# jolars/sgdnet

Measured on AMD Instinct MI355X. Metric: saga_epochs_per_sec, higher is better.
Workload: dtype f64

## Files before the change

### sgdnet_amd/csrc/saga_batched.hip

```cpp
#include <hip/hip_ext.h>
#include <stdlib.h>

#include <mutex>
#include <set>
#include <type_traits>
#include <utility>

#include "device_math.hpp"
#include "r_rng_word.hpp"
#include "r_rng_bodies.hpp"

#ifndef SGDNET_BIN_BLOCK
#define SGDNET_BIN_BLOCK 1024
#endif
#ifndef SGDNET_BIN_W
#define SGDNET_BIN_W 8
#endif
#ifndef SGDNET_RANGE_BLOCK
#define SGDNET_RANGE_BLOCK 512
#endif

namespace sgdnet {

namespace {
// ... 1615 lines not shown
  const int E = F * K;
  const int v = (int)blockIdx.x / nfb, fb = (int)blockIdx.x - v * nfb;
  const int64_t KP = (int64_t)K * d.p;
  const double n_d = d.v_size[v];
  const int e = threadIdx.x % kSlabElems, g = threadIdx.x / kSlabElems;
  const int64_t elem = (int64_t)fb * E + e;
  const int64_t j_own = (int64_t)fb * F + threadIdx.x;
  const bool updates = (int)threadIdx.x < F && j_own < d.p;
  double w_old[KMAX], g_old[KMAX], c_own = 0.0;
#pragma unroll
  for (int k = 0; k < KMAX; ++k) {
    w_old[k] = g_old[k] = 0.0;
    if (updates && k < K) {
      w_old[k] = d.vw[(int64_t)v * KP + j_own * K + k];
      g_old[k] = d.vG[(int64_t)v * KP + j_own * K + k];
    }
  }
  if (updates && d.standardize) c_own = d.c[j_own];
  double acc = 0.0;
  if (e < E && elem < KP) {
    const double* sp = d.slab + (int64_t)v * d.v_bps * KP + elem;
    int bidx = g;
    for (; bidx + 3 * kSlabGroups < d.v_bps; bidx += 4 * kSlabGroups) {
      const double a0 = sp[(int64_t)bidx * KP], a1 = sp[(int64_t)(bidx + kSlabGroups) * KP];
      const double a2 = sp[(int64_t)(bidx + 2 * kSlabGroups) * KP];
      const double a3 = sp[(int64_t)(bidx + 3 * kSlabGroups) * KP];
      acc += (a0 + a1) + (a2 + a3);
    }
    for (; bidx < d.v_bps; bidx += kSlabGroups) acc += sp[(int64_t)bidx * KP];
  }
  part[g][e] = acc;
  const bool need_d0 = fb == 0 || d.standardize;
  if (need_d0) {
    for (int k = 0; k < K; ++k) {
      double a = 0.0;
      for (int i = threadIdx.x; i < d.v_bps; i += kBlock) a += d.vd0[(int64_t)(v * d.v_bps + i) * K + k];
      a = wave_sum(a);
      if ((threadIdx.x & 63) == 0) red[threadIdx.x >> 6] = a;
      __syncthreads();
      if (threadIdx.x == 0) {
        double t = 0.0;
        for (int wv = 0; wv < kBlock / 64; ++wv) t += red[wv];
        sh_d0[k] = t;
      }
      __syncthreads();
    }
  } else {
    __syncthreads();
  }
  if (updates) {
    double dj[KMAX], val[KMAX];
#pragma unroll
    for (int k = 0; k < KMAX; ++k) {
      dj[k] = 0.0;
      if (k < K) {
        const int ee = (int)threadIdx.x * K + k;
        double t = 0.0;
        for (int gg = 0; gg < kSlabGroups; ++gg) t += part[gg][ee];
        dj[k] = t - (d.standardize ? c_own * sh_d0[k] : 0.0);
      }
    }
    const double gls = q.gamma * q.ls_m;
    double nrm = 0.0;
#pragma unroll
    for (int k = 0; k < KMAX; ++k) {
      val[k] = k < K ? q.r_m * w_old[k] - gls * g_old[k] - q.gamma * dj[k] : 0.0;
      nrm += val[k] * val[k];
    }
    const double tau = q.beta * q.gamma * q.ls_m;
    const double factor = q.penalty == SGDNET_GROUPLASSO ? tau / sqrt(nrm) : 0.0;
#pragma unroll
    for (int k = 0; k < KMAX; ++k) {
      if (k < K) {
        double out = val[k];
        if (q.penalty == SGDNET_ELASTICNET) out = soft_threshold(out, tau);
        else if (q.penalty == SGDNET_GROUPLASSO) out = factor < 1.0 ? out * (1.0 - factor) : 0.0;
        d.vw[(int64_t)v * KP + j_own * K + k] = out;
        if (dj[k] != 0.0 || q.penalty == SGDNET_GROUPLASSO)
          d.vG[(int64_t)v * KP + j_own * K + k] = g_old[k] + dj[k] / n_d;
      }
    }
  }
  if (fb == 0 && (int)threadIdx.x < K && d.fit_intercept) {
    const int k = threadIdx.x;
    const double dk = sh_d0[k] / n_d;
    const double gbk = d.vgb[v * K + k] + dk;
    d.vgb[v * K + k] = gbk;
    d.vb[v * K + k] -= q.gamma * (gbk * (d.xd ? 1.0 : 0.01) * q.m_d + dk);
  }
}

__global__ __launch_bounds__(kBlock) void saga_vs_cw_kernel(SagaDev d) {
  __shared__ double red[kBlock / 64];
  const int K = d.K;
  const int v = (int)blockIdx.x / K, k = (int)blockIdx.x - v * K;
  const double* wv = d.vw + (int64_t)v * K * d.p + k;
  double a = 0.0;
  for (int64_t j = threadIdx.x; j < d.p; j += kBlock) a += d.c[j] * wv[j * K];
  a = wave_sum(a);
  if ((threadIdx.x & 63) == 0) red[threadIdx.x >> 6] = a;
  __syncthreads();
  if (threadIdx.x == 0) {
    double t = 0.0;
    for (int wvi = 0; wvi < kBlock / 64; ++wvi) t += red[wvi];
    d.vcw[blockIdx.x] = t;
  }
}

__device__ __forceinline__ double* vs_slot(const SagaDev& d, int v, int64_t i, int64_t KP, int K) {
  if (i < KP) return d.vG + (int64_t)v * KP + i;
  if (i < 2 * KP) return d.vw + (int64_t)v * KP + (i - KP);
  if (i < 2 * KP + K) return d.vgb + (int64_t)v * K + (i - 2 * KP);
  return d.vb + (int64_t)v * K + (i - 2 * KP - K);
}
__device__ __forceinline__ double* vs_own_slot(const SagaDev& d, int64_t i, int64_t KP, int K) {
  if (i < KP) return d.G + i;
  if (i < 2 * KP) return d.w + (i - KP);
  if (i < 2 * KP + K) return d.gb + (i - 2 * KP);
  return d.b + (i - 2 * KP - K);
}

__global__ __launch_bounds__(kBlock) void saga_vs_broadcast_kernel(SagaDev d) {
  const int K = d.K;
  const int64_t KP = (int64_t)K * d.p, len = 2 * KP + 2 * K;
  for (int64_t i = (int64_t)blockIdx.x * kBlock + threadIdx.x; i < len; i += (int64_t)gridDim.x * kBlock) {
    const double val = *vs_own_slot(d, i, KP, K);
    d.vref[i] = val;
    for (int v = 0; v < d.V; ++v) *vs_slot(d, v, i, KP, K) = val;
  }
}

__global__ __launch_bounds__(kBlock) void saga_vs_merge_kernel(SagaDev d, int final_merge, LamParams* epoch_end,
                                                               int batches) {
  if (epoch_end && blockIdx.x == 0 && threadIdx.x == 0) end_epoch(epoch_end, batches);
  const int K = d.K;
  const int64_t KP = (int64_t)K * d.p, len = 2 * KP + 2 * K;
  double tot_size = 0.0;
  for (int v = 0; v < d.V; ++v) tot_size += d.v_size[v];
  for (int64_t i = (int64_t)blockIdx.x * kBlock + threadIdx.x; i < len; i += (int64_t)gridDim.x * kBlock) {
    const double ref = d.vref[i];
    double val = ref;
    for (int v = 0; v < d.V; ++v) val += (d.v_size[v] / tot_size) * (*vs_slot(d, v, i, KP, K) - ref);
    d.vref[i] = val;
    for (int v = 0; v < d.V; ++v) *vs_slot(d, v, i, KP, K) = val;
    if (final_merge) *vs_own_slot(d, i, KP, K) = val;
  }
}

__global__ void saga_epoch_end_kernel(LamParams* lamp, int batches) {
  if (threadIdx.x == 0 && blockIdx.x == 0) end_epoch(lamp, batches);
}

constexpr int kSyncLine = 32;
constexpr int kSyncGo = 0, kSyncExit = 1, kSyncStart = 2, kSyncCnt1 = 3, kSyncCnt2 = kSyncCnt1 + 8,
              kSyncXcd = kSyncCnt2 + 8;
constexpr int kFusedMaxBps = 128;
constexpr int kSyncLines = kSyncXcd + 8;
constexpr int kSyncSticky = kSyncLines;
constexpr int kSyncSeq = kSyncLines + 1;
constexpr int kFusedChunks = 3;
constexpr long long kFusedStartTicks = 2000000;
constexpr long long kFusedWaitTicks = 200000000;

typedef unsigned int u32x4_t __attribute__((ext_vector_type(4)));
typedef double f64x2_t __attribute__((ext_vector_type(2)));

__device__ __forceinline__ __amdgpu_buffer_rsrc_t fused_rsrc(const void* base, int64_t bytes) {
  return __builtin_amdgcn_make_buffer_rsrc(const_cast<void*>(base), 0, (int)bytes, 0x00020000);
}
__device__ __forceinline__ void st2_sc1(f64x2_t x, __amdgpu_buffer_rsrc_t rs, uint32_t byte_off) {
  __builtin_amdgcn_raw_buffer_store_b128(__builtin_bit_cast(u32x4_t, x), rs, (int)byte_off, 0, 16);
}
__device__ __forceinline__ f64x2_t ld2_sc1(__amdgpu_buffer_rsrc_t rs, uint32_t byte_off) {
  return __builtin_bit_cast(f64x2_t, __builtin_amdgcn_raw_buffer_load_b128(rs, (int)byte_off, 0, 16));
}
__device__ __forceinline__ void st2_shard(f64x2_t x, __amdgpu_buffer_rsrc_t rs, uint32_t byte_off, bool local) {
  if (local)
    __builtin_amdgcn_raw_buffer_store_b128(__builtin_bit_cast(u32x4_t, x), rs, (int)byte_off, 0, 0);
  else
    __builtin_amdgcn_raw_buffer_store_b128(__builtin_bit_cast(u32x4_t, x), rs, (int)byte_off, 0, 16);
}
__device__ __forceinline__ void st_shard(double* q, double x, bool local) {
  if (local)
    *q = x;
  else
    __hip_atomic_store(q, x, __ATOMIC_RELAXED, __HIP_MEMORY_SCOPE_AGENT);
}
__device__ __forceinline__ void st_sc1(double* q, double x) {
  __hip_atomic_store(q, x, __ATOMIC_RELAXED, __HIP_MEMORY_SCOPE_AGENT);
}
__device__ __forceinline__ double ld_sc1(const double* q) {
  return __hip_atomic_load(q, __ATOMIC_RELAXED, __HIP_MEMORY_SCOPE_AGENT);
}
__device__ __forceinline__ void st_sys(double* q, double x) {
  __hip_atomic_store(q, x, __ATOMIC_RELAXED, __HIP_MEMORY_SCOPE_SYSTEM);
}
__device__ __forceinline__ double ld_sys(const double* q) {
  return __hip_atomic_load(q, __ATOMIC_RELAXED, __HIP_MEMORY_SCOPE_SYSTEM);
}
__device__ __forceinline__ unsigned sync_load(unsigned* sync, int word) {
  return __hip_atomic_load(sync + word * kSyncLine, __ATOMIC_RELAXED, __HIP_MEMORY_SCOPE_AGENT);
}

__device__ __forceinline__ void fused_arrive(unsigned* sync, int word) {
  asm volatile("s_waitcnt vmcnt(0)" ::: "memory");
  __syncthreads();
  if (threadIdx.x == 0)
    __hip_atomic_fetch_add(sync + word * kSyncLine, 1u, __ATOMIC_RELAXED, __HIP_MEMORY_SCOPE_AGENT);
}

__device__ __forceinline__ bool fused_poll(unsigned* ctr, int word, unsigned target, LamParams* lamp, bool system = false,
                                           unsigned* sync = nullptr) {
  if (!sync) sync = ctr;
  const long long t0 = wall_clock64();
  for (unsigned spins = 1;; ++spins) {
    const unsigned now = system ? __hip_atomic_load(ctr + word * kSyncLine, __ATOMIC_RELAXED, __HIP_MEMORY_SCOPE_SYSTEM)
                                : sync_load(ctr, word);
    if (now >= target) return true;
    __builtin_amdgcn_s_sleep(4);
    if ((spins & 63u) == 0) {
      if (sync_load(sync, kSyncGo) != 1u) return false;
      if (wall_clock64() - t0 > kFusedWaitTicks) {
        __hip_atomic_store(sync + kSyncGo * kSyncLine, 3u, __ATOMIC_RELAXED, __HIP_MEMORY_SCOPE_AGENT);
        __hip_atomic_store(&lamp->fused_abort, 2, __ATOMIC_RELAXED, __HIP_MEMORY_SCOPE_AGENT);
        __hip_atomic_store(sync + kSyncSticky * kSyncLine, 2u, __ATOMIC_RELAXED, __HIP_MEMORY_SCOPE_AGENT);
        return false;
      }
    }
  }
}

__device__ __forceinline__ bool fused_start(unsigned* sync, LamParams* lamp, unsigned grid) {
  unsigned* go = sync + kSyncGo * kSyncLine;
  const long long t0 = wall_clock64();
  if (blockIdx.x == 0) {
    unsigned expect = 0u;
    for (;;) {
      if (sync_load(sync, kSyncStart) >= grid) {
        __hip_atomic_compare_exchange_strong(go, &expect, 1u, __ATOMIC_RELAXED, __ATOMIC_RELAXED, __HIP_MEMORY_SCOPE_AGENT);
        break;
      }
      if (sync_load(sync, kSyncGo) != 0u) break;
      if (wall_clock64() - t0 > kFusedStartTicks) {
        __hip_atomic_compare_exchange_strong(go, &expect, 2u, __ATOMIC_RELAXED, __ATOMIC_RELAXED, __HIP_MEMORY_SCOPE_AGENT);
        break;
      }
      __builtin_amdgcn_s_sleep(4);
    }
  } else {
    for (;;) {
      if (sync_load(sync, kSyncGo) != 0u) break;
      if (wall_clock64() - t0 > 2 * kFusedStartTicks) {
        unsigned expect = 0u;
        __hip_atomic_compare_exchange_strong(go, &expect, 2u, __ATOMIC_RELAXED, __ATOMIC_RELAXED, __HIP_MEMORY_SCOPE_AGENT);
        break;
      }
      __builtin_amdgcn_s_sleep(4);
    }
  }
  const unsigned decision = sync_load(sync, kSyncGo);
  if (decision != 1u && decision != 3u) {
    __hip_atomic_store(&lamp->fused_abort, 1, __ATOMIC_RELAXED, __HIP_MEMORY_SCOPE_AGENT);
    __hip_atomic_fetch_max(sync + kSyncSticky * kSyncLine, 1u, __ATOMIC_RELAXED, __HIP_MEMORY_SCOPE_AGENT);
  }
  return decision == 1u;
}

__device__ __forceinline__ double fused_block_sum(double a, double* red) {
  a = wave_sum(a);
  if ((threadIdx.x & 63) == 0) red[threadIdx.x >> 6] = a;
  __syncthreads();
  double t = 0.0;
#pragma unroll
  for (int wv = 0; wv < kLdsBlock / 64; ++wv) t += red[wv];
  __syncthreads();
  return t;
}

__device__ __forceinline__ void fused_leave(const SagaDev& d, LamParams* lamp, int nb, bool epoch_done) {
  asm volatile("s_waitcnt vmcnt(0)" ::: "memory");
  __syncthreads();
  if (threadIdx.x == 0) {
    unsigned* sync = d.vsync;
    if (epoch_done && blockIdx.x == 0) {
      end_epoch(lamp, nb);
      if (d.n_peers > 1) __hip_atomic_fetch_add(sync + kSyncSeq * kSyncLine, 1u, __ATOMIC_RELAXED, __HIP_MEMORY_SCOPE_AGENT);
    }
    const unsigned prev = __hip_atomic_fetch_add(sync + kSyncExit * kSyncLine, 1u, __ATOMIC_RELAXED, __HIP_MEMORY_SCOPE_AGENT);
    if (prev + 1u == gridDim.x) {
      for (int wd = 0; wd < kSyncLines; ++wd)
        __hip_atomic_store(sync + wd * kSyncLine, 0u, __ATOMIC_RELAXED, __HIP_MEMORY_SCOPE_AGENT);
      if (!(d.n_peers > 1))
        for (int wd = 0; wd < kFusedMaxBps; ++wd)
          __hip_atomic_store(d.vcol + wd * kSyncLine, 0u, __ATOMIC_RELAXED, __HIP_MEMORY_SCOPE_AGENT);
      if (d.rngdev && lamp->rng_generate) d.rngdev->gen += 1u;
    }
  }
}

template <bool kPeers>
__global__ __launch_bounds__(kLdsBlock) void saga_vs_epoch_kernel(SagaDev d, LamParams* lamp, int nb, int every) {
  extern __shared__ __attribute__((aligned(16))) double Dl[];
  __shared__ int ticket_counter;
  __shared__ int sh_ok;
  __shared__ double sh_red[kLdsBlock / 64];
  __shared__ double sh_val[4];
  const int tid = threadIdx.x;
  const int64_t p = d.p;
  const int64_t P2 = p >> 1;
  const int S = d.v_bps, V = d.V;
  if ((int)blockIdx.x >= V * S) {
    if (d.rngdev && lamp->rng_generate) {
      const RngDev* R = d.rngdev;
      const unsigned gen = R->gen;
      uint32_t* lds = reinterpret_cast<uint32_t*>(Dl);
      const int rb = (int)blockIdx.x - V * S, nrb = (int)gridDim.x - V * S;
      mt_state_body(rb, nrb, reinterpret_cast<uint32_t(*)[2][kMtN + 1]>(lds), R->state[gen & 1u], R->ends,
                    R->stream + (int64_t)(gen & 1u) * R->n, R->n, R->seg, R->gens);
      __syncthreads();
      mt_jump_body(rb, nrb, lds, R->state[gen & 1u], R->state[(gen + 1u) & 1u], R->poly, R->gens);
    }
    fused_leave(d, lamp, nb, false);
    return;
  }
  const int v = (int)blockIdx.x % V, wi = (int)blockIdx.x / V;
  const int F = 2 * (int)((p + 2 * S - 1) / (2 * S));
  const int j0 = wi * F;
  const int jn = p - j0 < F ? (p - j0 > 0 ? (int)(p - j0) : 0) : F;
  double* Wl = Dl + p;
  f64x2_t* D2 = reinterpret_cast<f64x2_t*>(Dl);
  f64x2_t* W2 = reinterpret_cast<f64x2_t*>(Wl);
  const int penalty = lamp->penalty;
  __shared__ double sh_par[10];
  if (tid == 0) {
    sh_par[0] = lamp->gamma;
    sh_par[1] = lamp->beta;
    sh_par[2] = lamp->r_full;
    sh_par[3] = lamp->ls_full;
    sh_par[4] = lamp->r_tail;
    sh_par[5] = lamp->ls_tail;
    double tot = 0.0, lo = 0.0;
    for (int u = 0; u < d.V; ++u) {
      tot += d.v_size[u];
      if (u < (int)blockIdx.x % d.V) lo += d.v_size[u];
    }
    sh_par[6] = d.v_size[(int)blockIdx.x % d.V];
    sh_par[7] = lo;
    sh_par[8] = tot;
  }
  const int64_t m_full = lamp->m_full;
  const int64_t sbase = lamp->stream_base;
  const bool raw_words = lamp->stream_raw != 0;
  const int64_t dps = d.v_dps;
  const bool std_x = d.standardize != 0;
  const int64_t L = 2 * p + 2;
  double* vwv = d.vw + (int64_t)v * p;
  double* vGv = d.vG + (int64_t)v * p;
  double* refv = d.vx + (int64_t)v * L;
  double* cwp = d.vx + (int64_t)V * L;
  unsigned* sync = d.vsync;
  const __amdgpu_buffer_rsrc_t rs_slab = fused_rsrc(d.slab, (int64_t)V * S * p * 8);
  const __amdgpu_buffer_rsrc_t rs_w = fused_rsrc(vwv, p * 8);
  uint32_t* const stream_v = const_cast<uint32_t*>(d.stream) + sbase + (int64_t)v * dps;
  constexpr int kC = 8;
  auto conv_range = [&](int m, int& lo, int& hi) {
    const int share = ((m + S - 1) / S + kTicket - 1) / kTicket * kTicket;
    lo = wi * share;
    hi = lo + share < m ? lo + share : m;
  };
  auto conv_load = [&](int64_t t0, int m, uint32_t (&x)[kC]) {
    int lo, hi;
    conv_range(m, lo, hi);
    const uint32_t* q = stream_v + t0;
#pragma unroll
    for (int c = 0; c < kC; ++c) {
      const int i = lo + (int)threadIdx.x + c * kLdsBlock;
      x[c] = i < hi ? q[i] : 0u;
    }
  };
  auto conv_store = [&](int64_t t0, int m, const uint32_t (&x)[kC]) {
    int lo, hi;
    conv_range(m, lo, hi);
    uint32_t* q = stream_v + t0;
    const double n_d = sh_par[6], lo_v = sh_par[7];
#pragma unroll
    for (int c = 0; c < kC; ++c) {
      const int i = lo + (int)threadIdx.x + c * kLdsBlock;
      if (i < hi) q[i] = (uint32_t)lo_v + word_to_draw(x[c], n_d);
    }
    for (int i = lo + (int)threadIdx.x + kC * kLdsBlock; i < hi; i += kLdsBlock)
      q[i] = (uint32_t)lo_v + word_to_draw(q[i], n_d);
  };

#ifdef SGDNET_PHASE_TIMING
  unsigned long long ph_t = 0;
  if (d.dbg && tid == 0) d.dbg[(size_t)blockIdx.x * 16 + 14] = ph_t = phase_stamp();
#define FPH(slot)                                                 \
  do {                                                            \
    if (d.dbg && tid == 0) {                                      \
      const unsigned long long now = phase_stamp();               \
      d.dbg[(size_t)blockIdx.x * 16 + (slot)] += now - ph_t;      \
      d.dbg[(size_t)blockIdx.x * 16 + 15] = ph_t = now;           \
    }                                                             \
  } while (0)
#else
#define FPH(slot) ((void)0)
#endif
  if (tid == 0) {
    const unsigned xcc = __builtin_amdgcn_s_getreg((3 << 11) | 20) & 15u;
    __hip_atomic_fetch_or(sync + (kSyncXcd + v) * kSyncLine, 1u << xcc, __ATOMIC_RELAXED, __HIP_MEMORY_SCOPE_AGENT);
    asm volatile("s_waitcnt vmcnt(0)" ::: "memory");
    __hip_atomic_fetch_add(sync + kSyncStart * kSyncLine, 1u, __ATOMIC_RELAXED, __HIP_MEMORY_SCOPE_AGENT);
    sh_ok = fused_start(sync, lamp, (unsigned)(V * S)) ? 1 : 0;
    if (sh_ok) {
      const unsigned mask = sync_load(sync, kSyncXcd + v);
      sh_ok = (mask & (mask - 1u)) == 0u ? 3 : 1;
    }
  }
  for (int64_t i = tid; i < P2; i += kLdsBlock) D2[i] = f64x2_t{0.0, 0.0};
  __syncthreads();
  bool done = false;
  bool alive = sh_ok != 0;
  unsigned col_base = 0u;
  if (kPeers) {
    int merges = 0;
    for (int r = 0; r < nb; ++r) merges += (r + 1 == nb || (r + 1) % every == 0) ? 1 : 0;
    col_base = sync_load(sync, kSyncSeq) * (unsigned)merges;
  }
  const bool local = (sh_ok & 2) != 0 && d.vs_xcd_local != 0;
  int mi = 0;
  uint32_t s_first = 0u, s_second = 0u;
  if (alive) {
    const int m0 = (int)(dps < m_full ? dps : m_full);
    if (raw_words) {
      uint32_t x0[kC];
      conv_load(0, m0, x0);
      conv_store(0, m0, x0);
      asm volatile("s_waitcnt vmcnt(0)" ::: "memory");
      __syncthreads();
    }
    K1Compact nx;
    nx.begin(d, stream_v, m0, wi, S, &ticket_counter);
    s_first = nx.s_cur;
    s_second = nx.s_nxt;
  }
  for (int r = 0; alive && r < nb; ++r) {
    const int64_t t0 = (int64_t)r * m_full;
    const int m = (int)(dps - t0 < m_full ? dps - t0 : m_full);
    const bool tail = m != m_full;
    const bool last = r + 1 == nb;
    const bool merge_due = last || (r + 1) % every == 0;

    if (tid == 0) ticket_counter = K1Compact::static_tickets();
    K1Compact cg;
    cg.init(d, stream_v + t0, m, wi, S, &ticket_counter);
    cg.s_cur = s_first;
    cg.s_nxt = s_second;
    cg.tag_first();
    int ts = threadIdx.x;
    asm volatile("" : "+v"(ts));
    double cw = 0.0, bv = 0.0;
    if ((ts >> 6) == 0) {
      if (std_x && r > 0)
        for (int k = ts & 63; k < S; k += 64) cw += ld_sc1(cwp + v * kFusedMaxBps + k);
      bv = r == 0 ? d.b[0] : ld_sc1(d.vb + v);
    }
    {
      constexpr int kStage = 8;
      for (int64_t i0 = ts; i0 < P2; i0 += (int64_t)kLdsBlock * kStage) {
        f64x2_t t[kStage];
#pragma unroll
        for (int q = 0; q < kStage; ++q) {
          const int64_t i = i0 + (int64_t)q * kLdsBlock;
          t[q] = f64x2_t{0.0, 0.0};
          if (i < P2) t[q] = r == 0 ? reinterpret_cast<const f64x2_t*>(d.w)[i] : ld2_sc1(rs_w, (uint32_t)(i * 16));
        }
#pragma unroll
        for (int q = 0; q < kStage; ++q) {
          const int64_t i = i0 + (int64_t)q * kLdsBlock;
          if (i < P2) W2[i] = t[q];
        }
      }
    }
    if ((ts >> 6) == 0) {
      cw = wave_sum(cw);
      if ((ts & 63) == 0) sh_val[0] = bv - cw;
    }
    __syncthreads();
    if (r == 0 && std_x) {
      double a = 0.0;
      for (int64_t j = ts; j < p; j += kLdsBlock) a += d.c[j] * Wl[j];
      a = fused_block_sum(a, sh_red);
      if (ts == 0) sh_val[0] -= a;
      __syncthreads();
    }
    const double b0 = sh_val[0];
    FPH(0);

    const double gct = cg.run(d, b0, Wl, Dl);
    __syncthreads();
    FPH(1);
    int tq = threadIdx.x;
    asm volatile("" : "+v"(tq));
    const int lane = tq & 63, wave = tq >> 6;
    const int64_t t0n = t0 + m_full;
    const int mn = (int)(dps - t0n < m_full ? dps - t0n : m_full);
    uint32_t xraw[kC];
    const bool conv_next = !last && raw_words;

    {
      const uint32_t base = (uint32_t)(((int64_t)blockIdx.x * p) * 8);
      for (int64_t i = tq; i < P2; i += kLdsBlock) {
        st2_shard(D2[i], rs_slab, base + (uint32_t)(i * 16), local);
        D2[i] = f64x2_t{0.0, 0.0};
      }
      const double t = wave_sum(gct);
      if (lane == 0) sh_red[wave] = t;
      __syncthreads();
      if (tq == 0) {
        double tot = 0.0;
        for (int wv = 0; wv < kLdsBlock / 64; ++wv) tot += sh_red[wv];
        st_shard(d.vd0 + blockIdx.x, tot, local);
      }
    }
    fused_arrive(sync, kSyncCnt1 + v);
    FPH(2);
    if (conv_next) conv_load(t0n, mn, xraw);
    const bool upd = tq < jn;
    const bool icpt = wi == 0 && tq == jn;
    const bool act = upd || icpt;
    const int64_t j = j0 + tq;
    const int64_t oa = upd ? j : 2 * p, ob = upd ? p + j : 2 * p + 1;
    double* const rep_a = upd ? vGv + j : d.vgb + v;
    double* const rep_b = upd ? vwv + j : d.vb + v;
    const double* const own_a = upd ? d.G + j : d.gb;
    const double* const own_b = upd ? d.w + j : d.b;
    double a_old = 0.0, b_old = 0.0, c_own = 0.0, ra = 0.0, rb = 0.0;
    if (act) {
      a_old = r == 0 ? *own_a : ld_sc1(rep_a);
      b_old = r == 0 ? *own_b : ld_sc1(rep_b);
      if (std_x && upd) c_own = d.c[j];
      if (merge_due) {
        ra = mi == 0 ? *own_a : ld_sc1(refv + oa);
        rb = mi == 0 ? *own_b : ld_sc1(refv + ob);
      }
    }
    if (tq == 0) sh_ok = fused_poll(sync, kSyncCnt1 + v, (unsigned)S * (unsigned)(r + 1), lamp) ? 1 : 0;
    __syncthreads();
    if (!sh_ok) break;
    FPH(3);
    if (conv_next) conv_store(t0n, mn, xraw);

    {
      double gsum = 0.0;
      if (wave == kLdsBlock / 64 - 1)
        for (int k = lane; k < S; k += 64) gsum += ld_sc1(d.vd0 + k * V + v);
      f64x2_t acc[kFusedChunks];
#pragma unroll
      for (int c = 0; c < kFusedChunks; ++c) acc[c] = f64x2_t{0.0, 0.0};
      for (int k = wave; k < S; k += 2 * (kLdsBlock / 64)) {
        const bool two = k + kLdsBlock / 64 < S;
        const uint32_t o0 = (uint32_t)((((int64_t)(k * V + v)) * p + j0) * 8);
        const uint32_t o1 = (uint32_t)((((int64_t)((k + kLdsBlock / 64) * V + v)) * p + j0) * 8);
        f64x2_t a0[kFusedChunks], a1[kFusedChunks];
#pragma unroll
        for (int c = 0; c < kFusedChunks; ++c) {
          const int pi = c * 64 + lane;
          a0[c] = a1[c] = f64x2_t{0.0, 0.0};
          if (2 * pi < jn) {
            a0[c] = ld2_sc1(rs_slab, o0 + (uint32_t)(pi * 16));
            if (two) a1[c] = ld2_sc1(rs_slab, o1 + (uint32_t)(pi * 16));
          }
        }
#pragma unroll
        for (int c = 0; c < kFusedChunks; ++c) {
          acc[c] += a0[c];
          acc[c] += a1[c];
        }
      }
#pragma unroll
      for (int c = 0; c < kFusedChunks; ++c) {
        const int pi = c * 64 + lane;
        if (2 * pi < F) reinterpret_cast<f64x2_t*>(Wl + (int64_t)wave * F)[pi] = acc[c];
      }
      if (wave == kLdsBlock / 64 - 1) {
        gsum = wave_sum(gsum);
        if (lane == 0) sh_val[1] = gsum;
      }
    }
    __syncthreads();
    double a_new = a_old, b_new = b_old;
    {
      const double d0 = sh_val[1];
      const double n_d = sh_par[6], gamma = sh_par[0];
      if (upd) {
        double dj = 0.0;
#pragma unroll
        for (int wv = 0; wv < kLdsBlock / 64; ++wv) dj += Wl[(int64_t)wv * F + tq];
        if (std_x) dj -= c_own * d0;
        const double beta = sh_par[1];
        const double r_m = tail ? sh_par[4] : sh_par[2], ls_m = tail ? sh_par[5] : sh_par[3];
        const double val = r_m * b_old - (gamma * ls_m) * a_old - gamma * dj;
        const double tau = beta * gamma * ls_m;
        b_new = val;
        if (penalty == SGDNET_ELASTICNET) {
          b_new = soft_threshold(val, tau);
        } else if (penalty == SGDNET_GROUPLASSO) {
          const double factor = tau / sqrt(val * val);
          b_new = factor < 1.0 ? val * (1.0 - factor) : 0.0;
        }
        a_new = (dj != 0.0 || penalty == SGDNET_GROUPLASSO) ? a_old + dj / n_d : a_old;
      } else if (icpt && d.fit_intercept) {
        const double dk = d0 / n_d;
        a_new = a_old + dk;
        b_new = b_old - gamma * (a_new * (d.xd ? 1.0 : 0.01) * (double)m + dk);
      }
    }
    FPH(4);
    if (merge_due) {
      const FusedPeers* PR = kPeers ? d.peers : nullptr;
      const int NP = kPeers ? d.n_peers : 1;
      double* pubv = d.vpub + (int64_t)((mi & 1) * V + v) * L;
      if (PR) {
        if (act) {
          st_sys(pubv + oa, a_new);
          st_sys(pubv + ob, b_new);
        }
        asm volatile("s_waitcnt vmcnt(0)" ::: "memory");
        __syncthreads();
        if (tq == 0)
          for (int q = 0; q < NP; ++q)
            __hip_atomic_fetch_add(PR->sync[q] + wi * kSyncLine, 1u, __ATOMIC_RELAXED, __HIP_MEMORY_SCOPE_SYSTEM);
      } else {
        if (act) {
          st_sc1(pubv + oa, a_new);
          st_sc1(pubv + ob, b_new);
        }
        fused_arrive(d.vcol, wi);
      }
      if (tq == 0)
        sh_ok = fused_poll(d.vcol, wi, (unsigned)(NP * V) * (col_base + (unsigned)(mi + 1)), lamp, PR != nullptr, sync) ? 1 : 0;
      __syncthreads();
      if (!sh_ok) break;
      double ma = ra, mb = rb;
      const double tot_all = PR ? PR->tot_size : sh_par[8];
      for (int q = 0; q < NP; ++q) {
        const double* pub0 = (PR ? PR->pub[q] : d.vpub) + (int64_t)((mi & 1) * V) * L;
        double xa[8], xb[8];
#pragma unroll
        for (int u = 0; u < 8; ++u) {
          xa[u] = xb[u] = 0.0;
          if (u < V && act) {
            xa[u] = PR ? ld_sys(pub0 + (int64_t)u * L + oa) : ld_sc1(pub0 + (int64_t)u * L + oa);
            xb[u] = PR ? ld_sys(pub0 + (int64_t)u * L + ob) : ld_sc1(pub0 + (int64_t)u * L + ob);
          }
        }
#pragma unroll
        for (int u = 0; u < 8; ++u) {
          if (u < V) {
            const double wt = (PR ? PR->vsize[q][u] : d.v_size[u]) / tot_all;
            ma += wt * (xa[u] - ra);
            mb += wt * (xb[u] - rb);
          }
        }
      }
      if (act) {
        a_new = ma;
        b_new = mb;
        st_sc1(refv + oa, ma);
        st_sc1(refv + ob, mb);
        if (last && v == 0) {
          *const_cast<double*>(own_a) = ma;
          *const_cast<double*>(own_b) = mb;
        }
      }
      ++mi;
      FPH(5);
    }
    if (act) {
      st_shard(rep_a, a_new, local);
      st_shard(rep_b, b_new, local);
    }
    if (std_x) {
      const double a = fused_block_sum(upd ? c_own * b_new : 0.0, sh_red);
      if (tq == 0) st_shard(cwp + v * kFusedMaxBps + wi, a, local);
    }
    if (last) {
      done = true;
      break;
    }
    fused_arrive(sync, kSyncCnt2 + v);
    FPH(6);
    {
      K1Compact nx;
      nx.begin(d, stream_v + t0n, mn, wi, S, &ticket_counter);
      s_first = nx.s_cur;
      s_second = nx.s_nxt;
    }
    if (tq == 0) sh_ok = fused_poll(sync, kSyncCnt2 + v, (unsigned)S * (unsigned)(r + 1), lamp) ? 1 : 0;
    __syncthreads();
    if (!sh_ok) break;
    FPH(7);
  }

  fused_leave(d, lamp, nb, done);
}

__global__ __launch_bounds__(kBlock) void saga_convergence_kernel(SagaDev d, LamParams* lamp) {
  const int64_t len = (int64_t)d.K * d.p;
  double max_change = 0.0, max_size = 0.0;
  for (int64_t i = (int64_t)blockIdx.x * kBlock + threadIdx.x; i < len; i += (int64_t)gridDim.x * kBlock) {
    const double v = d.w[i];
    max_change = fmax(max_change, fabs(v - d.w_prev[i]));
    max_size = fmax(max_size, fabs(v));
    d.w_prev[i] = v;
  }
  max_change = wave_max(max_change);
  max_size = wave_max(max_size);
  if ((threadIdx.x & 63) == 0) {
    atomic_max_bits(&lamp->max_change_bits, max_change);
    atomic_max_bits(&lamp->max_size_bits, max_size);
  }
}

template <bool kSparse>
__global__ __launch_bounds__(kBlock) void saga_loss_kernel(SagaDev d, LamParams* lamp) {
  extern __shared__ __attribute__((aligned(16))) char smem[];
  double* lps = reinterpret_cast<double*>(smem);
  const int K = d.K;
  const int gl = threadIdx.x & (kGroup - 1);
  const int gib = threadIdx.x / kGroup;
  const int64_t group = ((int64_t)blockIdx.x * kBlock + threadIdx.x) / kGroup;
  const int64_t ngroups = (int64_t)gridDim.x * (kBlock / kGroup);
  double* lp = lps + (size_t)gib * K;
  double* cw = lps + (size_t)(kBlock / kGroup) * K;
  if (kSparse && d.standardize) {
    __shared__ double red[kBlock / 64];
    for (int k = 0; k < K; ++k) {
      double a = 0.0;
      for (int64_t j = threadIdx.x; j < d.p; j += kBlock) a += d.w[k + j * K] * d.c[j];
      a = wave_sum(a);
      if ((threadIdx.x & 63) == 0) red[threadIdx.x >> 6] = a;
      __syncthreads();
      if (threadIdx.x == 0) {
        double t = 0.0;
        for (int wv = 0; wv < kBlock / 64; ++wv) t += red[wv];
        cw[k] = t;
      }
      __syncthreads();
    }
  }
  double loss = 0.0;
  if (kSparse && K > 1 && K <= kGroup) {
    const int kl = gl < K ? gl : 0;
    const double off = (gl < K ? d.b[kl] : 0.0) - (d.standardize ? cw[kl] : 0.0);
    for (int64_t s = group; s < d.n; s += ngroups) {
      const int64_t q0 = d.ptr[s], q1 = d.ptr[s + 1];
      double acc = 0.0;
      for (int64_t q = q0; q < q1; q += 4) {
        double xv[4];
        int64_t jv[4];
#pragma unroll
        for (int u = 0; u < 4; ++u) {
          xv[u] = q + u < q1 ? d.val[q + u] : 0.0;
          jv[u] = q + u < q1 ? (int64_t)d.idx[q + u] : 0;
        }
#pragma unroll
        for (int u = 0; u < 4; ++u) acc += xv[u] * d.w[kl + jv[u] * K];
      }
      if (gl < K) lp[gl] = acc + off;
      __builtin_amdgcn_wave_barrier();
      if (gl == 0) loss += family_loss(d.family, K, lp, d.y + s * d.Ky);
      __builtin_amdgcn_wave_barrier();
    }
    loss = wave_sum(loss);
    if ((threadIdx.x & 63) == 0 && loss != 0.0) atomic_add_f64(&lamp->loss_acc, loss);
    return;
  }
  for (int64_t s = group; s < d.n; s += ngroups) {
    for (int k = 0; k < K; ++k) {
      double acc = 0.0;
      if (kSparse) {
        for (int64_t q = d.ptr[s] + gl; q < d.ptr[s + 1]; q += kGroup)
          acc += d.val[q] * d.w[k + (int64_t)d.idx[q] * K];
      } else {
        for (int64_t j = gl; j < d.p; j += kGroup) acc += d.xd[s * d.p + j] * d.w[k + j * K];
      }
      acc = group_sum(acc);
      if (gl == 0) lp[k] = acc - (kSparse && d.standardize ? cw[k] : 0.0) + d.b[k];
    }
    __builtin_amdgcn_wave_barrier();
    if (gl == 0) loss += family_loss(d.family, K, lp, d.y + s * d.Ky);
    __builtin_amdgcn_wave_barrier();
  }
  loss = wave_sum(loss);
  if ((threadIdx.x & 63) == 0 && loss != 0.0) atomic_add_f64(&lamp->loss_acc, loss);
}

__global__ __launch_bounds__(kBlock) void saga_delta_export_kernel(SagaDev d, const double* ref,
                                                                   double* out, double weight) {
  const int64_t KP = (int64_t)d.K * d.p;
  const int64_t len = 2 * KP + 2 * d.K;
  for (int64_t i = (int64_t)blockIdx.x * kBlock + threadIdx.x; i < len; i += (int64_t)gridDim.x * kBlock) {
    double cur;
    if (i < KP) cur = d.G[i];
    else if (i < 2 * KP) cur = d.w[i - KP];
    else if (i < 2 * KP + d.K) cur = d.gb[i - 2 * KP];
    else cur = d.b[i - 2 * KP - d.K];
    out[i] = weight * (cur - ref[i]);
  }
}

__global__ __launch_bounds__(kBlock) void saga_delta_apply_kernel(SagaDev d, double* ref, const double* merged,
                                                                  double w_weight) {
  const int64_t KP = (int64_t)d.K * d.p;
  const int64_t len = 2 * KP + 2 * d.K;
  for (int64_t i = (int64_t)blockIdx.x * kBlock + threadIdx.x; i < len; i += (int64_t)gridDim.x * kBlock) {
    const bool coef = (i >= KP && i < 2 * KP) || i >= 2 * KP + d.K;
    const double v = ref[i] + (coef ? w_weight : 1.0) * merged[i];
    ref[i] = v;
    if (i < KP) d.G[i] = v;
    else if (i < 2 * KP) d.w[i - KP] = v;
    else if (i < 2 * KP + d.K) d.gb[i - 2 * KP] = v;
    else d.b[i - 2 * KP - d.K] = v;
  }
}

struct __attribute__((aligned(16))) BinEntry {
  uint32_t t;
  uint32_t j;
  double x;
};
static_assert(sizeof(BinEntry) == 16, "bin entries are 16 bytes");

constexpr int kBinBlock = SGDNET_BIN_BLOCK;
constexpr int kBinDraws = kBinBlock / 2;
constexpr int kBinEntCap = 7 * kBinBlock;
constexpr int kBinW = SGDNET_BIN_W;
constexpr int kRangeBlock = SGDNET_RANGE_BLOCK;
constexpr size_t kRangeLdsBytes = 64 * 1024;

size_t binned_max_range_features(int K) { return kRangeLdsBytes / (sizeof(double) * (size_t)K); }

__global__ __launch_bounds__(256) void col_count_kernel(const int32_t* idx, int64_t nnz, unsigned* counts) {
  for (int64_t q = (int64_t)blockIdx.x * 256 + threadIdx.x; q < nnz; q += (int64_t)gridDim.x * 256)
    atomicAdd(counts + idx[q], 1u);
}

__global__ __launch_bounds__(256) void wpad_refresh_kernel(const double* w, double* wpad, int K, int KS, int64_t p) {
  const int64_t t = (int64_t)blockIdx.x * 256 + threadIdx.x;
  if (t < p * KS) {
    const int64_t j = t / KS;
    const int k = (int)(t - j * KS);
    wpad[t] = k < K ? w[j * K + k] : 0.0;
// ... 387 lines not shown
    }
#pragma unroll
    for (int qq = 0; qq < kEnt; ++qq) {
      const int j = __shfl((int)mine.j, qq, kGrp);
      const double x = shfl_d<kGrp>(mine.x, qq);
      if (lane_on && e0 + qq < cntb) scatter_add<true>(Dl + (j - lo) * K + gl, x * gq[qq]);
    }
    mine = nxt;
  }
  PHASE(8);
  __syncthreads();
  PHASE(9);
  if (threadIdx.x == 0) d.bin_count[r] = 0u;
  if (kGrouped) {
    double cwp[kGrp];
    for (int k = 0; k < K; ++k) cwp[k] = 0.0;
    for (int f = threadIdx.x; f < hi - lo; f += kRangeBlock) {
      const int64_t j = lo + f;
      double dj[kGrp], wn[kGrp];
      const double cj = d.standardize ? d.c[j] : 0.0;
      for (int k = 0; k < K; ++k) dj[k] = Dl[f * K + k] - (d.standardize ? cj * sh_d0[k] : 0.0);
      sweep_feature(d, q, j, dj, wn);
      for (int k = 0; k < K; ++k) cwp[k] += cj * wn[k];
      if (d.wpad != d.w)
        for (int k = 0; k < K; ++k) d.wpad[j * d.KS + k] = wn[k];
    }
    if (d.standardize) cw_accumulate<kRangeBlock>(d, batch_id, cwp);
  } else {
    const double tau = q.beta * q.gamma * q.ls_m, gls = q.gamma * q.ls_m;
    if (d.standardize) {
      if ((int)threadIdx.x < kGrp) sh_cw[threadIdx.x] = 0.0;
      __syncthreads();
    }
    for (int i = threadIdx.x; i < E; i += kRangeBlock) {
      const int f = i / K, k = i - f * K;
      const int64_t t = (int64_t)lo * K + i;
      const double cj = d.standardize ? d.c[lo + f] : 0.0;
      const double dk = Dl[i] - (d.standardize ? cj * sh_d0[k] : 0.0);
      double v = q.r_m * d.w[t] - gls * d.G[t] - q.gamma * dk;
      if (q.penalty == SGDNET_ELASTICNET) v = soft_threshold(v, tau);
      d.w[t] = v;
      if (d.wpad != d.w) d.wpad[(int64_t)(lo + f) * d.KS + k] = v;
      if (dk != 0.0) d.G[t] += dk / q.n_d;
      if (d.standardize && cj * v != 0.0)
        __hip_atomic_fetch_add(&sh_cw[k], cj * v, __ATOMIC_RELAXED, __HIP_MEMORY_SCOPE_WORKGROUP);
    }
    if (d.standardize) {
      __syncthreads();
      if ((int)threadIdx.x < K) {
        const double tot = sh_cw[threadIdx.x];
        double* set = d.cw + (size_t)((batch_id + 1) & 1) * kCwSlots * K;
        if (tot != 0.0) atomic_add_f64(set + (blockIdx.x % kCwSlots) * K + threadIdx.x, tot);
      }
    }
  }
  PHASE(10);
}

int batched_max_classes() { return 64; }

int lds_target_grid(const SagaDev& d) {
  static const int forced = exp_env_int("SGDNET_LDS_GRID", 0);
  if (forced > 0) return forced;
  const int cus = d.cu_budget > 0 && d.cu_budget < 256 ? d.cu_budget : 256;
  const int g = cus - d.cu_reserve;
  return g < 64 ? 64 : g;
}

constexpr size_t kLdsPerCu = 160 * 1024;
constexpr size_t kLdsStaticReserve = 2 * 1024;
constexpr size_t kLdsTableMax = 80 * 1024;
constexpr int kLdsCap = 96 * 1024;
constexpr int kLdsAll = (int)(kLdsPerCu - kLdsStaticReserve);
constexpr int kDenseVsBlock = 1024;

static size_t table_bytes(const SagaDev& d) { return sizeof(double) * (size_t)d.K * (size_t)d.p; }

int allow_dynamic_lds(const void* kernel, int bytes) {
  int dev = 0;
  (void)hipGetDevice(&dev);
  static std::mutex mu;
  static std::set<std::pair<const void*, int>> done;
  std::lock_guard<std::mutex> lock(mu);
  if (done.count({kernel, dev})) return SGDNET_OK;
  SGD_HIP_TRY(hipFuncSetAttribute(kernel, hipFuncAttributeMaxDynamicSharedMemorySize, bytes));
  done.insert({kernel, dev});
  return SGDNET_OK;
}

static int class_width(int K) { return K == 1 ? 1 : K <= 4 ? 4 : K <= 16 ? 16 : 64; }

template <typename F>
static int with_class_width(int kw, F&& f) {
  if (kw == 1) return f(std::integral_constant<int, 1>{});
  if (kw == 4) return f(std::integral_constant<int, 4>{});
  return f(std::integral_constant<int, 16>{});
}

static bool lanes8_ok(const SagaDev& d) {
  static const int allow = exp_env_int("SGDNET_LANES8", 1);
  return allow && (d.cP || d.rec_cap >= kInReg8) && !SGD_ABLATE(d, ~0);
}

bool compact_eligible(const SagaDev& d) {
  static const int allow = exp_env_int("SGDNET_COMPACT", 1);
  if (!allow || d.K != 1 || d.Ky != 1 || d.xd || !d.ptr || d.p > 65536) return false;
  if (2 * sizeof(double) * (size_t)d.p + 16 + kLdsStaticReserve > (size_t)kLdsPerCu) return false;
  return (double)d.n * 2.0 * kCStride <= 48e9 && d.n < (int64_t)kIdMask;
}

int compact_entries(const SagaDev& d) { return d.family == SGDNET_BINOMIAL && d.y_binary ? 12 : 11; }

int launch_pack_compact(const SagaDev& d, char* P, char* Q, uint32_t* meta, hipStream_t st) {
  SGD_HIP_TRY(hipMemsetAsync(meta, 0, sizeof(uint32_t) * (size_t)((d.n + 15) / 16 + 1), st));
  int64_t grid = (d.n + 255) / 256;
  if (grid > 65536) grid = 65536;
  const int E = compact_entries(d);
  hipLaunchKernelGGL(pack_compact_kernel, dim3((unsigned)grid), dim3(256), 0, st, d.ptr, d.idx, d.val, d.y, d.n, E,
                     E == 12 ? 1 : 0, P, Q, meta);
  SGD_HIP_TRY(hipGetLastError());
  return SGDNET_OK;
}

int launch_m_move(const SagaDev& d, int to_record, hipStream_t st) {
  int64_t grid = (d.n + 255) / 256;
  if (grid > 16384) grid = 16384;
  hipLaunchKernelGGL(m_move_kernel, dim3((unsigned)grid), dim3(256), 0, st, d, to_record);
  SGD_HIP_TRY(hipGetLastError());
  return SGDNET_OK;
}
bool wants_binned(const SagaDev& d, int64_t batch) {
  static const int allow = exp_env_int("SGDNET_BINNED", 1);
  return allow && !d.xd && d.rec && d.idx && d.K <= 64 && !d.force_global && d.p < (1ll << 31) &&
         (d.K > 16 || (table_bytes(d) > kLdsTableMax && batch >= 4096));
}

bool wants_tiles(const SagaDev& d) { return d.xd && d.K <= 64 && (d.K > 16 || table_bytes(d) > kLdsTableMax); }

bool vs_eligible(const SagaDev& d) {
  if (d.V < 2 || d.K < 1 || d.K > 16 || (d.standardize && !(d.vcw && d.c)) || d.force_global || !d.vw) return false;
  const size_t table = table_bytes(d);
  if (d.xd) return table <= kLdsTableMax;
  if (d.K > 1) return d.rec && table <= kLdsTableMax;
  return 2 * table + 16 + kLdsStaticReserve <= kLdsPerCu;
}

static int vs_grid(const SagaDev& d) { return d.v_bps * d.V; }

static int64_t fused_slice(const SagaDev& d) { return 2 * ((d.p + 2 * (int64_t)d.v_bps - 1) / (2 * (int64_t)d.v_bps)); }
static size_t fused_lds_bytes(const SagaDev& d) {
  const int64_t part = (int64_t)(kLdsBlock / 64) * fused_slice(d);
  return sizeof(double) * (size_t)(d.p + (part > d.p ? part : d.p)) + 16;
}
size_t vs_fused_sync_words() { return (size_t)(kSyncLines + 2) * kSyncLine; }
size_t vs_fused_sync_sticky_word() { return (size_t)kSyncSticky * kSyncLine; }
size_t vs_fused_col_words() { return (size_t)kFusedMaxBps * kSyncLine; }
size_t vs_fused_exchange_doubles(const SagaDev& d, int n_shards) {
  return (size_t)n_shards * (size_t)(2 * d.p + 2) + (size_t)n_shards * kFusedMaxBps;
}
size_t vs_fused_publish_doubles(const SagaDev& d, int n_shards) { return (size_t)2 * n_shards * (size_t)(2 * d.p + 2); }

bool vs_fused_eligible(const SagaDev& d) {
  if (!vs_eligible(d) || d.K != 1 || d.xd || !d.cP || !lanes8_ok(d) || (d.p & 1) || !d.vsync || !d.vx || !d.vcol || !d.vpub) return false;
  if (d.v_bps < 1 || d.v_bps > kFusedMaxBps || d.V * d.v_bps > 1024) return false;
  if (fused_slice(d) > 2 * 64 * kFusedChunks) return false;
  if ((int64_t)d.V * d.v_bps * d.p * 8 >= (1ll << 31)) return false;
  return fused_lds_bytes(d) + kLdsStaticReserve <= kLdsPerCu;
}

static int vs_fused_rng_workgroups(const SagaDev& d) { return d.rngdev ? d.cu_reserve : 0; }

BatchPlan plan_batch(const SagaDev& d, int m, const PlanInputs& in) {
  BatchPlan g{};
  g.kw = class_width(d.K);
  const size_t table = table_bytes(d);
  if (d.V > 1 && vs_eligible(d)) {
    const int rng_wgs = vs_fused_rng_workgroups(d);
    g.slab_doubles = (int64_t)vs_grid(d) * d.K * d.p;
    if (in.fused && vs_fused_eligible(d) && vs_grid(d) + rng_wgs <= in.cus) {
      g.form = BatchForm::kFusedEpoch;
      g.grid = vs_grid(d) + rng_wgs;
      g.lds_bytes = fused_lds_bytes(d);
      if (rng_wgs > 0 && g.lds_bytes < kJumpLds) g.lds_bytes = kJumpLds;
      return g;
    }
    g.form = BatchForm::kShards;
    g.grid = vs_grid(d);
    int dpb = (m + d.v_bps - 1) / d.v_bps;
    g.lds_bytes = table;
    if (d.xd) {
      const int waves = (d.K > 1 ? kDenseBlock : kDenseVsBlock) / 64;
      dpb = (dpb + waves - 1) / waves * waves;
    } else {
      const int per_round = kLdsBlock / kGroup;
      if (dpb < per_round) dpb = per_round;
      if (d.K == 1) {
        g.w_lds = true;
        g.lanes8 = lanes8_ok(d);
        g.lds_bytes = 2 * table + 16;
      }
    }
    g.draws_per_block = dpb;
    return g;
  }
  static const int force = [] {
    const char* e = exp_env_str("SGDNET_GATHER");
    return !e ? 0 : (e[0] == 'l' ? 1 : 2);
  }();
  const int target_grid = lds_target_grid(d);
  const bool fits = table <= kLdsTableMax;
  if (d.xd) {
    const int waves = kDenseBlock / 64;
    if (wants_tiles(d)) {
      g.form = d.K > 16 ? BatchForm::kDenseClassLane : BatchForm::kDenseTiled;
      int dpb = (m + 8191) / 8192;
      dpb = (dpb + waves - 1) / waves * waves;
      if (dpb < waves) dpb = waves;
      g.draws_per_block = dpb;
      g.grid = (m + dpb - 1) / dpb;
      if (g.grid < 1) g.grid = 1;
      const int64_t tiles = (d.p + kTileF - 1) / kTileF;
      int64_t chunks = (2048 + tiles - 1) / tiles;
      const int64_t most = (m + 4 * waves - 1) / (4 * waves);
      if (chunks > most) chunks = most;
      if (chunks < 1) chunks = 1;
      if (chunks > 65535) chunks = 65535;
      g.draws_per_chunk = (int)((m + chunks - 1) / chunks);
      g.chunks = (int)((m + g.draws_per_chunk - 1) / g.draws_per_chunk);
      g.slab_doubles = fits ? (int64_t)g.grid * d.K * d.p : 0;
      return g;
    }
    g.form = BatchForm::kDense;
    int dpb = (m + target_grid - 1) / target_grid;
    dpb = (dpb + waves - 1) / waves * waves;
    if (dpb < waves) dpb = waves;
    g.draws_per_block = dpb;
    g.grid = (m + dpb - 1) / dpb;
    if (g.grid < 1) g.grid = 1;
    g.lds_bytes = table;
    g.slab_doubles = fits ? (int64_t)g.grid * d.K * d.p : 0;
    return g;
  }
  if (wants_binned(d, in.batch) && d.R > 0 && !in.bins_disabled && force != 2 && m <= (1 << 20)) {
    g.form = BatchForm::kBinned;
    g.draws_per_block = kBinDraws;
    g.grid = (m + kBinDraws - 1) / kBinDraws;
    if (g.grid < 1) g.grid = 1;
    g.lds_bytes = sizeof(BinEntry) * (size_t)kBinEntCap + sizeof(unsigned) * (3 * (size_t)d.R + 1) +
                  ((sizeof(unsigned short) * ((size_t)d.n_coarse + 1) + 15) & ~size_t(15));
    return g;
  }
  const bool pays = (double)m * (double)d.avg_nnz >= 48.0 * (double)d.K * (double)d.p;
  if (!d.force_global && fits && force != 2 && (force == 1 || pays)) {
    g.form = BatchForm::kLds;
    int dpb = (m + target_grid - 1) / target_grid;
    const int per_round = kLdsBlock / kGroup;
    if (dpb < per_round) dpb = per_round;
    g.draws_per_block = dpb;
    g.grid = (m + dpb - 1) / dpb;
    g.lds_bytes = table;
    static const bool w_lds_on = exp_env_int("SGDNET_W_LDS", 1) != 0;
    g.w_lds = d.K == 1 && w_lds_on && 2 * table + kLdsStaticReserve <= kLdsPerCu;
    if (g.w_lds) g.lds_bytes = 2 * table + 16;
    g.lanes8 = g.w_lds && lanes8_ok(d);
  } else {
    g.form = BatchForm::kGlobal;
    g.draws_per_block = kBlock / kGroup;
    g.grid = (m + g.draws_per_block - 1) / g.draws_per_block;
  }
  if (g.grid < 1) g.grid = 1;
  if (g.form == BatchForm::kLds) g.slab_doubles = (int64_t)g.grid * d.K * d.p;
  return g;
}

int launch_batch_gather(const SagaDev& d, const BatchPlan& g, LamParams* lam, int64_t t0_in_epoch, int m,
                        int batch_id_offset, hipStream_t st, hipEvent_t ev0, hipEvent_t ev1) {
  if (d.K > 16 && g.form != BatchForm::kBinned && g.form != BatchForm::kDenseClassLane) {
    set_error("batched mode with more than 16 classes needs the binned form (sparse x) or the class-lane form (dense x), "
              "n_classes <= 64; got %d", d.K);
    return SGDNET_EUNSUPPORTED;
  }
  const dim3 agrid((unsigned)((d.p + kTileF - 1) / kTileF), (unsigned)g.chunks, (unsigned)((d.K + 15) / 16));
  switch (g.form) {
  case BatchForm::kDenseClassLane:
    hipExtLaunchKernelGGL(saga_dense_cl_gather_kernel, dim3(g.grid), dim3(kDenseBlock), 0, st, ev0, nullptr, 0, d, lam,
                          t0_in_epoch, m, batch_id_offset, g.draws_per_block);
    SGD_HIP_TRY(hipGetLastError());
    hipExtLaunchKernelGGL(saga_dense_tiled_accumulate_kernel<16>, agrid, dim3(kDenseBlock), 0, st, nullptr, ev1, 0, d, lam,
                          t0_in_epoch, m, g.draws_per_chunk);
    break;
  case BatchForm::kDenseTiled:
    return with_class_width(g.kw, [&](auto kw) {
      constexpr int KW = decltype(kw)::value;
      hipExtLaunchKernelGGL((saga_batch_gather_dense_kernel<KW, kDenseBlock, false, true>), dim3(g.grid), dim3(kDenseBlock),
                            0, st, ev0, nullptr, 0, d, lam, t0_in_epoch, m, batch_id_offset, g.draws_per_block);
      SGD_HIP_TRY(hipGetLastError());
      hipExtLaunchKernelGGL(saga_dense_tiled_accumulate_kernel<KW>, agrid, dim3(kDenseBlock), 0, st, nullptr, ev1, 0, d,
                            lam, t0_in_epoch, m, g.draws_per_chunk);
      SGD_HIP_TRY(hipGetLastError());
      return SGDNET_OK;
    });
  case BatchForm::kDense:
    return with_class_width(g.kw, [&](auto kw) {
      constexpr int KW = decltype(kw)::value;
      const int rc = allow_dynamic_lds(saga_batch_gather_dense_kernel<KW>, kLdsCap);
      if (rc) return rc;
      hipExtLaunchKernelGGL(saga_batch_gather_dense_kernel<KW>, dim3(g.grid), dim3(kDenseBlock), g.lds_bytes, st,
// ... 230 lines not shown
```

Measured before the change: 1156.

## Replace fused-kernel counter barriers with per-block epoch stamps and point-to-point waits

The two grid-wide counter barriers in the fused SAGA epoch kernel are replaced by per-workgroup stamp lines. Each block publishes its round number once its slab or slice is written, and consumers wait only on the specific producer stamps they read, using wave-wide polling with __all. At the start of each round every block now reloads the weight slices chunk by chunk after checking each producer's stamp, instead of copying the whole weight vector after a full barrier. The aim is to remove global barrier latency and let blocks overlap. In exchange the sync buffer grows, a persistent rounds counter is added, and memory-ordering correctness rests on relaxed atomics plus waitcnt fences.

```diff
diff --git a/sgdnet_amd/csrc/saga_batched.hip b/sgdnet_amd/csrc/saga_batched.hip
--- a/sgdnet_amd/csrc/saga_batched.hip
+++ b/sgdnet_amd/csrc/saga_batched.hip
@@ -1791,12 +1791,15 @@
 }
 
 constexpr int kSyncLine = 32;
-constexpr int kSyncGo = 0, kSyncExit = 1, kSyncStart = 2, kSyncCnt1 = 3, kSyncCnt2 = kSyncCnt1 + 8,
-              kSyncXcd = kSyncCnt2 + 8;
+constexpr int kSyncGo = 0, kSyncExit = 1, kSyncStart = 2, kSyncXcd = 3;
 constexpr int kFusedMaxBps = 128;
 constexpr int kSyncLines = kSyncXcd + 8;
 constexpr int kSyncSticky = kSyncLines;
 constexpr int kSyncSeq = kSyncLines + 1;
+constexpr int kSyncRounds = kSyncLines + 2;
+constexpr int kSyncSlab = kSyncLines + 3;
+constexpr int kSyncSlice = kSyncSlab + 8 * kFusedMaxBps;
+constexpr int kSyncAll = kSyncSlice + 8 * kFusedMaxBps;
 constexpr int kFusedChunks = 3;
 constexpr long long kFusedStartTicks = 2000000;
 constexpr long long kFusedWaitTicks = 200000000;
@@ -1869,6 +1872,37 @@
   }
 }
 
+__device__ __forceinline__ void fused_stamp(unsigned* sync, int line, unsigned value) {
+  asm volatile("s_waitcnt vmcnt(0)" ::: "memory");
+  __syncthreads();
+  if (threadIdx.x == 0) __hip_atomic_store(sync + line * kSyncLine, value, __ATOMIC_RELAXED, __HIP_MEMORY_SCOPE_AGENT);
+}
+
+__device__ __forceinline__ bool stamps_wait(unsigned* sync, int line, bool mine, unsigned target, LamParams* lamp) {
+  const long long t0 = wall_clock64();
+  bool ok = true;
+  for (unsigned spins = 1;; ++spins) {
+    const unsigned now = mine ? sync_load(sync, line) : target;
+    if (__all((int)(now - target) >= 0)) break;
+    __builtin_amdgcn_s_sleep(4);
+    if ((spins & 63u) == 0) {
+      if (sync_load(sync, kSyncGo) != 1u) {
+        ok = false;
+        break;
+      }
+      if (wall_clock64() - t0 > kFusedWaitTicks) {
+        __hip_atomic_store(sync + kSyncGo * kSyncLine, 3u, __ATOMIC_RELAXED, __HIP_MEMORY_SCOPE_AGENT);
+        __hip_atomic_store(&lamp->fused_abort, 2, __ATOMIC_RELAXED, __HIP_MEMORY_SCOPE_AGENT);
+        __hip_atomic_store(sync + kSyncSticky * kSyncLine, 2u, __ATOMIC_RELAXED, __HIP_MEMORY_SCOPE_AGENT);
+        ok = false;
+        break;
+      }
+    }
+  }
+  asm volatile("" ::: "memory");
+  return ok;
+}
+
 __device__ __forceinline__ bool fused_start(unsigned* sync, LamParams* lamp, unsigned grid) {
   unsigned* go = sync + kSyncGo * kSyncLine;
   const long long t0 = wall_clock64();
@@ -1929,6 +1963,7 @@
     if (prev + 1u == gridDim.x) {
       for (int wd = 0; wd < kSyncLines; ++wd)
         __hip_atomic_store(sync + wd * kSyncLine, 0u, __ATOMIC_RELAXED, __HIP_MEMORY_SCOPE_AGENT);
+      __hip_atomic_fetch_add(sync + kSyncRounds * kSyncLine, (unsigned)nb, __ATOMIC_RELAXED, __HIP_MEMORY_SCOPE_AGENT);
       if (!(d.n_peers > 1))
         for (int wd = 0; wd < kFusedMaxBps; ++wd)
           __hip_atomic_store(d.vcol + wd * kSyncLine, 0u, __ATOMIC_RELAXED, __HIP_MEMORY_SCOPE_AGENT);
@@ -1944,6 +1979,7 @@
   __shared__ int sh_ok;
   __shared__ double sh_red[kLdsBlock / 64];
   __shared__ double sh_val[4];
+  __shared__ unsigned sh_stamp;
   const int tid = threadIdx.x;
   const int64_t p = d.p;
   const int64_t P2 = p >> 1;
@@ -2051,6 +2087,7 @@
     asm volatile("s_waitcnt vmcnt(0)" ::: "memory");
     __hip_atomic_fetch_add(sync + kSyncStart * kSyncLine, 1u, __ATOMIC_RELAXED, __HIP_MEMORY_SCOPE_AGENT);
     sh_ok = fused_start(sync, lamp, (unsigned)(V * S)) ? 1 : 0;
+    sh_stamp = sync_load(sync, kSyncRounds);
     if (sh_ok) {
       const unsigned mask = sync_load(sync, kSyncXcd + v);
       sh_ok = (mask & (mask - 1u)) == 0u ? 3 : 1;
@@ -2100,11 +2137,43 @@
     asm volatile("" : "+v"(ts));
     double cw = 0.0, bv = 0.0;
     if ((ts >> 6) == 0) {
+      if (r > 0) {
+        const unsigned tgt = sh_stamp + (unsigned)r;
+        bool ok = stamps_wait(sync, kSyncSlice + v * kFusedMaxBps + (ts & 63), (ts & 63) < S, tgt, lamp);
+        if (S > 64) ok = stamps_wait(sync, kSyncSlice + v * kFusedMaxBps + 64 + (ts & 63), 64 + (ts & 63) < S, tgt, lamp) && ok;
+        if (!ok) sh_ok = 0;
+      }
       if (std_x && r > 0)
         for (int k = ts & 63; k < S; k += 64) cw += ld_sc1(cwp + v * kFusedMaxBps + k);
       bv = r == 0 ? d.b[0] : ld_sc1(d.vb + v);
     }
-    {
+    if (r > 0) {
+      const int wave_s = ts >> 6, lane_s = ts & 63;
+      const unsigned tgt = sh_stamp + (unsigned)r;
+      for (int k = wave_s; k < S; k += 2 * (kLdsBlock / 64)) {
+        const int k1 = k + kLdsBlock / 64;
+        const int kw = lane_s == 0 ? k : k1;
+        if (wave_s != 0 &&
+            !stamps_wait(sync, kSyncSlice + v * kFusedMaxBps + kw, lane_s < 2 && kw < S && kw != wi, tgt, lamp))
+          sh_ok = 0;
+        f64x2_t t0v[kFusedChunks], t1v[kFusedChunks];
+        const int n0 = (int)(p - (int64_t)k * F < F ? p - (int64_t)k * F : F);
+        const int n1 = k1 < S ? (int)(p - (int64_t)k1 * F < F ? (p - (int64_t)k1 * F > 0 ? p - (int64_t)k1 * F : 0) : F) : 0;
+#pragma unroll
+        for (int c = 0; c < kFusedChunks; ++c) {
+          const int pi = c * 64 + lane_s;
+          t0v[c] = t1v[c] = f64x2_t{0.0, 0.0};
+          if (2 * pi < n0) t0v[c] = ld2_sc1(rs_w, (uint32_t)(((int64_t)k * F + 2 * pi) * 8));
+          if (2 * pi < n1) t1v[c] = ld2_sc1(rs_w, (uint32_t)(((int64_t)k1 * F + 2 * pi) * 8));
+        }
+#pragma unroll
+        for (int c = 0; c < kFusedChunks; ++c) {
+          const int pi = c * 64 + lane_s;
+          if (2 * pi < n0) W2[(int64_t)k * (F / 2) + pi] = t0v[c];
+          if (2 * pi < n1) W2[(int64_t)k1 * (F / 2) + pi] = t1v[c];
+        }
+      }
+    } else {
       constexpr int kStage = 8;
       for (int64_t i0 = ts; i0 < P2; i0 += (int64_t)kLdsBlock * kStage) {
         f64x2_t t[kStage];
@@ -2112,7 +2181,7 @@
         for (int q = 0; q < kStage; ++q) {
           const int64_t i = i0 + (int64_t)q * kLdsBlock;
           t[q] = f64x2_t{0.0, 0.0};
-          if (i < P2) t[q] = r == 0 ? reinterpret_cast<const f64x2_t*>(d.w)[i] : ld2_sc1(rs_w, (uint32_t)(i * 16));
+          if (i < P2) t[q] = reinterpret_cast<const f64x2_t*>(d.w)[i];
         }
 #pragma unroll
         for (int q = 0; q < kStage; ++q) {
@@ -2126,6 +2195,7 @@
       if ((ts & 63) == 0) sh_val[0] = bv - cw;
     }
     __syncthreads();
+    if (!sh_ok) break;
     if (r == 0 && std_x) {
       double a = 0.0;
       for (int64_t j = ts; j < p; j += kLdsBlock) a += d.c[j] * Wl[j];
@@ -2162,7 +2232,7 @@
         st_shard(d.vd0 + blockIdx.x, tot, local);
       }
     }
-    fused_arrive(sync, kSyncCnt1 + v);
+    fused_stamp(sync, kSyncSlab + v * kFusedMaxBps + wi, sh_stamp + (unsigned)(r + 1));
     FPH(2);
     if (conv_next) conv_load(t0n, mn, xraw);
     const bool upd = tq < jn;
@@ -2184,21 +2254,27 @@
         rb = mi == 0 ? *own_b : ld_sc1(refv + ob);
       }
     }
-    if (tq == 0) sh_ok = fused_poll(sync, kSyncCnt1 + v, (unsigned)S * (unsigned)(r + 1), lamp) ? 1 : 0;
-    __syncthreads();
-    if (!sh_ok) break;
     FPH(3);
     if (conv_next) conv_store(t0n, mn, xraw);
 
     {
+      const unsigned tgt = sh_stamp + (unsigned)(r + 1);
       double gsum = 0.0;
-      if (wave == kLdsBlock / 64 - 1)
+      if (wave == kLdsBlock / 64 - 1) {
+        bool ok = stamps_wait(sync, kSyncSlab + v * kFusedMaxBps + lane, lane < S, tgt, lamp);
+        if (S > 64) ok = stamps_wait(sync, kSyncSlab + v * kFusedMaxBps + 64 + lane, 64 + lane < S, tgt, lamp) && ok;
+        if (!ok) sh_ok = 0;
         for (int k = lane; k < S; k += 64) gsum += ld_sc1(d.vd0 + k * V + v);
+      }
       f64x2_t acc[kFusedChunks];
 #pragma unroll
       for (int c = 0; c < kFusedChunks; ++c) acc[c] = f64x2_t{0.0, 0.0};
       for (int k = wave; k < S; k += 2 * (kLdsBlock / 64)) {
         const bool two = k + kLdsBlock / 64 < S;
+        const int kw = lane == 0 ? k : k + kLdsBlock / 64;
+        if (wave != kLdsBlock / 64 - 1 &&
+            !stamps_wait(sync, kSyncSlab + v * kFusedMaxBps + kw, lane < 2 && kw < S && kw != wi, tgt, lamp))
+          sh_ok = 0;
         const uint32_t o0 = (uint32_t)((((int64_t)(k * V + v)) * p + j0) * 8);
         const uint32_t o1 = (uint32_t)((((int64_t)((k + kLdsBlock / 64) * V + v)) * p + j0) * 8);
         f64x2_t a0[kFusedChunks], a1[kFusedChunks];
@@ -2228,6 +2304,7 @@
       }
     }
     __syncthreads();
+    if (!sh_ok) break;
     double a_new = a_old, b_new = b_old;
     {
       const double d0 = sh_val[1];
@@ -2328,7 +2405,7 @@
       done = true;
       break;
     }
-    fused_arrive(sync, kSyncCnt2 + v);
+    fused_stamp(sync, kSyncSlice + v * kFusedMaxBps + wi, sh_stamp + (unsigned)(r + 1));
     FPH(6);
     {
       K1Compact nx;
@@ -2336,9 +2413,6 @@
       s_first = nx.s_cur;
       s_second = nx.s_nxt;
     }
-    if (tq == 0) sh_ok = fused_poll(sync, kSyncCnt2 + v, (unsigned)S * (unsigned)(r + 1), lamp) ? 1 : 0;
-    __syncthreads();
-    if (!sh_ok) break;
     FPH(7);
   }
 
@@ -3032,7 +3106,7 @@
   const int64_t part = (int64_t)(kLdsBlock / 64) * fused_slice(d);
   return sizeof(double) * (size_t)(d.p + (part > d.p ? part : d.p)) + 16;
 }
-size_t vs_fused_sync_words() { return (size_t)(kSyncLines + 2) * kSyncLine; }
+size_t vs_fused_sync_words() { return (size_t)kSyncAll * kSyncLine; }
 size_t vs_fused_sync_sticky_word() { return (size_t)kSyncSticky * kSyncLine; }
 size_t vs_fused_col_words() { return (size_t)kFusedMaxBps * kSyncLine; }
 size_t vs_fused_exchange_doubles(const SagaDev& d, int n_shards) {
```

Result: no change. 1159 (median of 6 runs) (+0.3%).
